# HarborC/PL-SLAM

Hardware: NVIDIA H100
Metric: frames/sec (extract+match+pose-LM) 640x480 (higher is better)
Workload: dtype u8/i32 front-end, f32 descriptors, f64 LM

## Files before the change

pl-slam_b200/csrc/match.cu:

```cuda

#include "common.cuh"
#include "search.cuh"
#include "libm_glibc.cuh"
#include <vector>

namespace pl {

constexpr int GC = 64, GR = 48, NCELL = GC * GR, HISTO = 30;

__device__ __forceinline__ int hamming256(const uint8_t* a, const uint8_t* b) {
  const uint4* pa = reinterpret_cast<const uint4*>(a);
  const uint4* pb = reinterpret_cast<const uint4*>(b);
  uint4 a0 = pa[0], a1 = pa[1], b0 = pb[0], b1 = pb[1];
  return __popc(a0.x ^ b0.x) + __popc(a0.y ^ b0.y) + __popc(a0.z ^ b0.z) + __popc(a0.w ^ b0.w) +
         __popc(a1.x ^ b1.x) + __popc(a1.y ^ b1.y) + __popc(a1.z ^ b1.z) + __popc(a1.w ^ b1.w);
}

__device__ __forceinline__ unsigned long long warp_min_u64(unsigned long long v) {
#pragma unroll
  for (int o = 16; o > 0; o >>= 1) {
    unsigned long long t = __shfl_xor_sync(0xffffffffu, v, o);
    v = t < v ? t : v;
  }
  return v;
}

struct GridP { float minX, minY, maxX, maxY, invW, invH; };
__host__ __device__ inline GridP make_grid(const float* b) {
  GridP g;
  g.minX = b[0]; g.minY = b[1]; g.maxX = b[2]; g.maxY = b[3];
  g.invW = (float)GC / (g.maxX - g.minX);
  g.invH = (float)GR / (g.maxY - g.minY);
  return g;
}

__device__ void build_point_grid(const PLKeyPoint* keys, int n, const GridP& g, unsigned short* start,
                                 unsigned short* fill, unsigned short* items, int lane) {
  for (int i = lane; i < NCELL; i += 32) fill[i] = 0;
  __syncwarp();
  for (int i0 = 0; i0 < n; i0 += 32) {
    int i = i0 + lane, c = -1;
    if (i < n) {
      int px = (int)roundf(__fmul_rn(__fsub_rn(keys[i].x, g.minX), g.invW));
      int py = (int)roundf(__fmul_rn(__fsub_rn(keys[i].y, g.minY), g.invH));
      if (px >= 0 && px < GC && py >= 0 && py < GR) c = px * GR + py;
    }
    unsigned peers = __match_any_sync(0xffffffffu, c);
    if (c >= 0 && (peers & ((1u << lane) - 1u)) == 0) fill[c] += (unsigned short)__popc(peers);
    __syncwarp();
  }
  int run = 0;
  for (int c0 = 0; c0 < NCELL; c0 += 32) {
    int v = fill[c0 + lane], incl = v;
#pragma unroll
    for (int o = 1; o < 32; o <<= 1) { int t = __shfl_up_sync(0xffffffffu, incl, o); if (lane >= o) incl += t; }
    start[c0 + lane] = (unsigned short)(run + incl - v);
    run += __shfl_sync(0xffffffffu, incl, 31);
  }
  if (lane == 0) start[NCELL] = (unsigned short)run;
  __syncwarp();
  for (int i = lane; i < NCELL; i += 32) fill[i] = 0;
  __syncwarp();
  for (int i0 = 0; i0 < n; i0 += 32) {
    int i = i0 + lane, c = -1;
    if (i < n) {
      int px = (int)roundf(__fmul_rn(__fsub_rn(keys[i].x, g.minX), g.invW));
      int py = (int)roundf(__fmul_rn(__fsub_rn(keys[i].y, g.minY), g.invH));
      if (px >= 0 && px < GC && py >= 0 && py < GR) c = px * GR + py;
    }
    unsigned peers = __match_any_sync(0xffffffffu, c);
    unsigned lt = peers & ((1u << lane) - 1u);
    if (c >= 0) items[start[c] + fill[c] + __popc(lt)] = (unsigned short)i;
    __syncwarp();
    if (c >= 0 && lt == 0) fill[c] += (unsigned short)__popc(peers);
    __syncwarp();
  }
}

struct Window { int x0, x1, y0, y1; bool ok; };
__device__ __forceinline__ Window make_window(const GridP& g, float x, float y, float r) {
  Window w;
  w.ok = false;
  w.x0 = max(0, (int)floorf(__fmul_rn(__fsub_rn(__fsub_rn(x, g.minX), r), g.invW)));
  if (w.x0 >= GC) return w;
  w.x1 = min(GC - 1, (int)ceilf(__fmul_rn(__fadd_rn(__fsub_rn(x, g.minX), r), g.invW)));
  if (w.x1 < 0) return w;
  w.y0 = max(0, (int)floorf(__fmul_rn(__fsub_rn(__fsub_rn(y, g.minY), r), g.invH)));
  if (w.y0 >= GR) return w;
  w.y1 = min(GR - 1, (int)ceilf(__fmul_rn(__fadd_rn(__fsub_rn(y, g.minY), r), g.invH)));
  if (w.y1 < 0) return w;
  w.ok = true;
  return w;
}

__device__ __forceinline__ unsigned long long mk_key(int dist, int c, int j, int idx) {
  return ((unsigned long long)dist << 52) | ((unsigned long long)c << 40) | ((unsigned long long)j << 20) |
         (unsigned long long)idx;
}
constexpr unsigned long long KEY_NONE = ~0ull;
__device__ __forceinline__ int key_dist(unsigned long long k) { return (int)(k >> 52); }
__device__ __forceinline__ int key_idx(unsigned long long k) { return (int)(k & 0xfffff); }

struct Top2 { unsigned long long best, second; };

constexpr int kPackShift = 11, kPackIdMask = (1 << kPackShift) - 1, kPackMaxKeys = 1 << kPackShift;
__device__ __forceinline__ bool pack_octaves(const PLKeyPoint* keys, int n, int nitems, unsigned short* items, int lane) {
  if (n > kPackMaxKeys) return false;
  for (int j = lane; j < nitems; j += 32) {
    const int id = items[j];
    items[j] = (unsigned short)(id | ((keys[id].octave & 31) << kPackShift));
  }
  __syncwarp();
  return true;
}

template <typename Skip>
__device__ __forceinline__ Top2 window_top2(const PLKeyPoint* keys, const uint8_t* desc, const unsigned short* start,
                                            const unsigned short* items, const GridP& g, float x, float y, float r,
                                            int minLevel, int maxLevel, const uint8_t* q, Skip skip, int lane,
                                            bool packed = false) {
  Top2 t;
  t.best = KEY_NONE; t.second = KEY_NONE;
  Window w = make_window(g, x, y, r);
  if (!w.ok) return t;
  const bool checkLevels = (minLevel > 0) || (maxLevel >= 0);
  const int ncy = w.y1 - w.y0 + 1, ncell = (w.x1 - w.x0 + 1) * ncy;
  unsigned long long k1 = KEY_NONE, k2 = KEY_NONE;
  const int q32 = 32 / ncy, r32 = 32 - q32 * ncy;
  int cx = lane / ncy, cy = lane - cx * ncy;
  for (int c = lane; c < ncell; c += 32, cx += q32, cy += r32) {
    if (cy >= ncy) { cy -= ncy; cx++; }
    const int ix = w.x0 + cx, iy = w.y0 + cy;
    int cb = start[ix * GR + iy], ce = start[ix * GR + iy + 1];
    for (int j = cb; j < ce; j++) {
      const int it = items[j];
      const int id = packed ? (it & kPackIdMask) : it;
      if (checkLevels) {
        const int oct = packed ? (it >> kPackShift) : keys[id].octave;
        if (oct < minLevel) continue;
        if (maxLevel >= 0 && oct > maxLevel) continue;
      }
      const PLKeyPoint& kp = keys[id];
      if (!(fabsf(__fsub_rn(kp.x, x)) < r && fabsf(__fsub_rn(kp.y, y)) < r)) continue;
      int dist = hamming256(q, desc + 32 * id);
      if (skip(id, dist)) continue;
      unsigned long long k = mk_key(dist, c, j - cb, id);
      if (k < k1) { k2 = k1; k1 = k; }
      else if (k < k2) k2 = k;
    }
  }
  t.best = warp_min_u64(k1);
  t.second = warp_min_u64(k1 == t.best ? k2 : k1);
  return t;
}

__device__ void three_maxima(const int* cnt, int& ind1, int& ind2, int& ind3) {
  int max1 = 0, max2 = 0, max3 = 0;
  ind1 = ind2 = ind3 = -1;
  for (int i = 0; i < HISTO; i++) {
    const int s = cnt[i];
    if (s > max1) { max3 = max2; max2 = max1; max1 = s; ind3 = ind2; ind2 = ind1; ind1 = i; }
    else if (s > max2) { max3 = max2; max2 = s; ind3 = ind2; ind2 = i; }
    else if (s > max3) { max3 = s; ind3 = i; }
  }
  if ((float)max2 < __fmul_rn(0.1f, (float)max1)) { ind2 = -1; ind3 = -1; }
  else if ((float)max3 < __fmul_rn(0.1f, (float)max1)) { ind3 = -1; }
}
__device__ __forceinline__ int rot_bin(float a1, float a2) {
  float rot = __fsub_rn(a1, a2);
  if (rot < 0.0f) rot = __fadd_rn(rot, 360.0f);
  int bin = (int)roundf(__fmul_rn(rot, 1.0f / HISTO));
  if (bin == HISTO) bin = 0;
  return bin;
}

struct SmemGrid {
  unsigned short* start; unsigned short* fill; unsigned short* items;
};
__device__ __forceinline__ SmemGrid carve_grid(unsigned char* smem, int cap) {
  SmemGrid s;
  s.start = reinterpret_cast<unsigned short*>(smem);
  s.fill = s.start + NCELL + 2;
  s.items = s.fill + NCELL;
  (void)cap;
  return s;
}
static size_t grid_smem_bytes(int cap) { return (size_t)(NCELL + 2 + NCELL + cap) * 2; }

__global__ void __launch_bounds__(32) k_assign_grid(const PLKeyPoint* keys, const int* n, int cap, const float* bounds,
                                                    int* out_start, int* out_items) {
  extern __shared__ unsigned char smem[];
  const int b = blockIdx.x, lane = threadIdx.x;
  SmemGrid sg = carve_grid(smem, cap);
  GridP g = make_grid(bounds);
  const int nn = min(n[b], cap);
  build_point_grid(keys + (long long)b * cap, nn, g, sg.start, sg.fill, sg.items, lane);
  __syncwarp();
  for (int i = lane; i <= NCELL; i += 32) out_start[(long long)b * (NCELL + 1) + i] = sg.start[i];
  for (int i = lane; i < sg.start[NCELL]; i += 32) out_items[(long long)b * cap + i] = sg.items[i];
}

struct SkipInit {
  const int* matchedDist;
  __device__ bool operator()(int id, int dist) const { return matchedDist[id] <= dist; }
};

__global__ void __launch_bounds__(32) k_search_init(const PLKeyPoint* keys1, const uint8_t* desc1, const int* n1,
                                                    const PLKeyPoint* keys2, const uint8_t* desc2, const int* n2,
                                                    int cap, const float* bounds, float* prev_matched, int* matches12,
                                                    int* nmatches_out, int windowSize, float nnratio, int checkOri,
                                                    int* scratch ) {
  extern __shared__ unsigned char smem[];
  __shared__ int hist[HISTO];
  const int b = blockIdx.x, lane = threadIdx.x;
  SmemGrid sg = carve_grid(smem, cap);
  GridP g = make_grid(bounds);
  const PLKeyPoint* k1 = keys1 + (long long)b * cap;
  const PLKeyPoint* k2 = keys2 + (long long)b * cap;
  const uint8_t* d1 = desc1 + (long long)b * cap * 32;
  const uint8_t* d2 = desc2 + (long long)b * cap * 32;
  const int N1 = min(n1[b], cap), N2 = min(n2[b], cap);
  float* pm = prev_matched + (long long)b * cap * 2;
  int* m12 = matches12 + (long long)b * cap;
  int* matchedDist = scratch + (long long)b * 2 * cap;
  int* m21 = matchedDist + cap;
  build_point_grid(k2, N2, g, sg.start, sg.fill, sg.items, lane);
  const bool packed = pack_octaves(k2, N2, sg.start[NCELL], sg.items, lane);
  for (int i = lane; i < N1; i += 32) m12[i] = -1;
  for (int i = lane; i < N2; i += 32) { matchedDist[i] = 0x7fffffff; m21[i] = -1; }
  if (lane < HISTO) hist[lane] = 0;
  __syncwarp();
  unsigned char* bins = reinterpret_cast<unsigned char*>(sg.fill);
  for (int i = lane; i < N1; i += 32) bins[i] = 255;
  __syncwarp();
  int nmatches = 0;
  SkipInit skip{matchedDist};
  for (int i1 = 0; i1 < N1; i1++) {
    if (k1[i1].octave > 0) continue;
    Top2 t = window_top2(k2, d2, sg.start, sg.items, g, pm[2 * i1], pm[2 * i1 + 1], (float)windowSize, 0, 0,
                         d1 + 32 * i1, skip, lane, packed);
    if (t.best == KEY_NONE) continue;
    const int bestDist = key_dist(t.best), bestIdx2 = key_idx(t.best);
    const float bestDist2 = (t.second == KEY_NONE) ? 2147483648.0f : (float)key_dist(t.second);
    if (bestDist <= 50 && (float)bestDist < __fmul_rn(bestDist2, nnratio)) {
      int old = m21[bestIdx2];
      __syncwarp();
      if (old >= 0) nmatches--;
      nmatches++;
      if (lane == 0) {
        if (old >= 0) m12[old] = -1;
        m12[i1] = bestIdx2;
        m21[bestIdx2] = i1;
        matchedDist[bestIdx2] = bestDist;
        if (checkOri) { int bin = rot_bin(k1[i1].angle, k2[bestIdx2].angle); bins[i1] = (unsigned char)bin; hist[bin]++; }
      }
      __syncwarp();
    }
  }
  if (checkOri) {
    int i1m, i2m, i3m;
    three_maxima(hist, i1m, i2m, i3m);
    int removed = 0;
    for (int i = lane; i < N1; i += 32) {
      int bin = bins[i];
      if (bin != 255 && bin != i1m && bin != i2m && bin != i3m && m12[i] >= 0) { m12[i] = -1; removed++; }
    }
    nmatches -= warp_sum(removed);
  }
  __syncwarp();
  for (int i = lane; i < N1; i += 32)
    if (m12[i] >= 0) { pm[2 * i] = k2[m12[i]].x; pm[2 * i + 1] = k2[m12[i]].y; }
  if (lane == 0) nmatches_out[b] = nmatches;
}

struct SkipAssigned {
  const int* match;
  __device__ bool operator()(int id, int) const { return match[id] != -1; }
};

struct ProjLastArgs {
  const PLKeyPoint* keys; const uint8_t* desc; const int* n; int cap;
  const float* bounds; const float* Tcw; const float* K; const float* scaleFactors; int nlevels;
  const int* n_last; int cap_last; const uint8_t* last_valid; const float* last_pos; const uint8_t* last_desc;
  const int* last_octave; const float* last_angle;
  float th; int checkOri; const uint8_t* preassigned; int* match; int* nmatches;
  int kfMode = 0, maxDist = 100; const float *min_dist = nullptr, *max_dist = nullptr; float Ow[3] = {0, 0, 0}; float logSF = 1.f;
  const int* gate = nullptr; int gate_min = 0;
  const int* last_row = nullptr;
};

__global__ void __launch_bounds__(32) k_search_proj_last(ProjLastArgs A) {
  extern __shared__ unsigned char smem[];
  __shared__ int hist[HISTO];
  const int b = blockIdx.x, lane = threadIdx.x;
  if (A.gate && A.gate[b] >= A.gate_min) return;
  SmemGrid sg = carve_grid(smem, A.cap);
  GridP g = make_grid(A.bounds);
  const PLKeyPoint* kc = A.keys + (long long)b * A.cap;
  const uint8_t* dc = A.desc + (long long)b * A.cap * 32;
  const int N = min(A.n[b], A.cap), NL = min(A.n_last[b], A.cap_last);
  int* match = A.match + (long long)b * A.cap;
  const float* T = A.Tcw + 16 * b;
  const long long lb = (long long)b * A.cap_last;
  build_point_grid(kc, N, g, sg.start, sg.fill, sg.items, lane);
  const bool packed = pack_octaves(kc, N, sg.start[NCELL], sg.items, lane);
  for (int i = lane; i < N; i += 32) match[i] = (A.preassigned && A.preassigned[(long long)b * A.cap + i]) ? -2 : -1;
  if (lane < HISTO) hist[lane] = 0;
  unsigned char* bins = reinterpret_cast<unsigned char*>(sg.fill);
  __syncwarp();
  for (int i = lane; i < N; i += 32) bins[i] = 255;
  __syncwarp();
  int nmatches = 0;
  SkipAssigned skip{match};
  const float* Kb = A.K + 4 * b;
  const float fx = Kb[0], fy = Kb[1], cx = Kb[2], cy = Kb[3];
  for (int i = 0; i < NL; i++) {
    if (!A.last_valid[lb + i]) continue;
    const long long row = A.last_row ? (long long)A.last_row[lb + i] : lb + i;
    const float* X = A.last_pos + row * 3;
    float xc = __fadd_rn(__fadd_rn(__fadd_rn(__fmul_rn(T[0], X[0]), __fmul_rn(T[1], X[1])), __fmul_rn(T[2], X[2])), T[3]);
    float yc = __fadd_rn(__fadd_rn(__fadd_rn(__fmul_rn(T[4], X[0]), __fmul_rn(T[5], X[1])), __fmul_rn(T[6], X[2])), T[7]);
    float zc = __fadd_rn(__fadd_rn(__fadd_rn(__fmul_rn(T[8], X[0]), __fmul_rn(T[9], X[1])), __fmul_rn(T[10], X[2])), T[11]);
    const float invzc = (float)(1.0 / (double)zc);
    if (!A.kfMode && invzc < 0) continue;
    float u = __fadd_rn(__fmul_rn(__fmul_rn(fx, xc), invzc), cx);
    float v = __fadd_rn(__fmul_rn(__fmul_rn(fy, yc), invzc), cy);
    if (u < g.minX || u > g.maxX) continue;
    if (v < g.minY || v > g.maxY) continue;
    int oct;
    if (A.kfMode) {
      const float p0 = __fsub_rn(X[0], A.Ow[0]), p1 = __fsub_rn(X[1], A.Ow[1]), p2 = __fsub_rn(X[2], A.Ow[2]);
      const float dist3D = (float)sqrt((double)p0 * p0 + (double)p1 * p1 + (double)p2 * p2);
      if (dist3D < __fmul_rn(0.8f, A.min_dist[lb + i]) || dist3D > __fmul_rn(1.2f, A.max_dist[lb + i])) continue;
      const float ratio = __fdiv_rn(A.max_dist[lb + i], dist3D);
      oct = (int)ceilf(__fdiv_rn(glibc::logf_(ratio), A.logSF));
      if (oct < 0) oct = 0; else if (oct >= A.nlevels) oct = A.nlevels - 1;
    } else oct = A.last_octave[lb + i];
    const float radius = __fmul_rn(A.th, A.scaleFactors[oct]);
    Top2 t = window_top2(kc, dc, sg.start, sg.items, g, u, v, radius, oct - 1, oct + 1, A.last_desc + row * 32,
                         skip, lane, packed);
    if (t.best == KEY_NONE) continue;
    const int bestDist = key_dist(t.best), bestIdx2 = key_idx(t.best);
    if (bestDist <= A.maxDist) {
      nmatches++;
      if (lane == 0) {
        match[bestIdx2] = i;
        if (A.checkOri) { int bin = rot_bin(A.last_angle[lb + i], kc[bestIdx2].angle); bins[bestIdx2] = (unsigned char)bin; hist[bin]++; }
      }
      __syncwarp();
    }
  }
  if (A.checkOri) {
    int i1m, i2m, i3m;
    three_maxima(hist, i1m, i2m, i3m);
    int removed = 0;
    for (int i = lane; i < N; i += 32) {
      int bin = bins[i];
      if (bin != 255 && bin != i1m && bin != i2m && bin != i3m) { match[i] = -1; removed++; }
    }
    nmatches -= warp_sum(removed);
  }
  if (lane == 0) A.nmatches[b] = nmatches;
}

struct ProjPointsArgs {
  const PLKeyPoint* keys; const uint8_t* desc; const int* n; int cap;
  const float* bounds; const float* scaleFactors;
  const int* n_mp; int cap_mp; const uint8_t* in_view; const float* proj; const int* level; const float* view_cos;
  const uint8_t* mp_desc; float th; float nnratio; const uint8_t* preassigned; int* match; int* nmatches;
  const float* th_frame;
  const int* desc_row;
};

__global__ void __launch_bounds__(32) k_search_proj_points(ProjPointsArgs A) {
  extern __shared__ unsigned char smem[];
  const int b = blockIdx.x, lane = threadIdx.x;
  SmemGrid sg = carve_grid(smem, A.cap);
  GridP g = make_grid(A.bounds);
  const PLKeyPoint* k = A.keys + (long long)b * A.cap;
  const uint8_t* d = A.desc + (long long)b * A.cap * 32;
  const int N = min(A.n[b], A.cap), NM = min(A.n_mp[b], A.cap_mp);
  int* match = A.match + (long long)b * A.cap;
  const long long mb = (long long)b * A.cap_mp;
  build_point_grid(k, N, g, sg.start, sg.fill, sg.items, lane);
  const bool packed = pack_octaves(k, N, sg.start[NCELL], sg.items, lane);
  for (int i = lane; i < N; i += 32) match[i] = (A.preassigned && A.preassigned[(long long)b * A.cap + i]) ? -2 : -1;
  __syncwarp();
  int nmatches = 0;
  SkipAssigned skip{match};
  const float th = A.th_frame ? A.th_frame[b] : A.th;
  const bool bFactor = th != 1.0f;
  for (int i = 0; i < NM; i++) {
    if (!A.in_view[mb + i]) continue;
    const int lvl = A.level[mb + i];
    float r = ((double)A.view_cos[mb + i] > 0.998) ? 2.5f : 4.0f;
    if (bFactor) r = __fmul_rn(r, th);
    const long long drow = A.desc_row ? (long long)A.desc_row[mb + i] : mb + i;
    Top2 t = window_top2(k, d, sg.start, sg.items, g, A.proj[(mb + i) * 2], A.proj[(mb + i) * 2 + 1],
                         __fmul_rn(r, A.scaleFactors[lvl]), lvl - 1, lvl, A.mp_desc + drow * 32, skip, lane, packed);
    if (t.best == KEY_NONE) continue;
    const int bestDist = key_dist(t.best), bestIdx = key_idx(t.best);
    if (bestDist <= 100) {
      if (t.second != KEY_NONE) {
        const int bestDist2 = key_dist(t.second);
        if (k[bestIdx].octave == k[key_idx(t.second)].octave && (float)bestDist > __fmul_rn(A.nnratio, (float)bestDist2))
          continue;
      }
      nmatches++;
      if (lane == 0) match[bestIdx] = i;
      __syncwarp();
    }
  }
  if (lane == 0) A.nmatches[b] = nmatches;
}

__device__ __forceinline__ void knn2_row(const uint8_t* q, const uint8_t* train, int n2, int lane, int& i0, int& d0,
                                         int& i1, int& d1v) {
  unsigned long long k1 = KEY_NONE, k2 = KEY_NONE;
  for (int t = lane; t < n2; t += 32) {
    unsigned long long k = ((unsigned long long)hamming256(q, train + 32 * t) << 32) | (unsigned)t;
    if (k < k1) { k2 = k1; k1 = k; } else if (k < k2) k2 = k;
  }
  unsigned long long b = warp_min_u64(k1);
  unsigned long long s = warp_min_u64(k1 == b ? k2 : k1);
  i0 = b == KEY_NONE ? -1 : (int)(b & 0xffffffffu); d0 = b == KEY_NONE ? -1 : (int)(b >> 32);
  i1 = s == KEY_NONE ? -1 : (int)(s & 0xffffffffu); d1v = s == KEY_NONE ? -1 : (int)(s >> 32);
}

__global__ void __launch_bounds__(128) k_bf_knn2(const uint8_t* d1, const int* n1, const uint8_t* d2, const int* n2,
                                                 int cap1, int cap2, int* idx, int* dist) {
  const int b = blockIdx.y, lane = threadIdx.x & 31, q = blockIdx.x * 4 + (threadIdx.x >> 5);
  const int N1 = min(n1[b], cap1), N2 = min(n2[b], cap2);
  if (q >= N1) return;
  int i0, dd0, i1, dd1;
  knn2_row(d1 + ((long long)b * cap1 + q) * 32, d2 + (long long)b * cap2 * 32, N2, lane, i0, dd0, i1, dd1);
  if (lane == 0) {
    long long o = ((long long)b * cap1 + q) * 2;
    idx[o] = i0; idx[o + 1] = i1; dist[o] = dd0; dist[o + 1] = dd1;
  }
}

__device__ void frame_bf_match_cta(const uint8_t* da, int na, const uint8_t* db, int nb, float TH, float nnratio,
                                   short* m, short* bd0, short* bd1, int* hist ) {
  const int tid = threadIdx.x, lane = tid & 31, wid = tid >> 5;
  for (int i = tid; i < na; i += 128) m[i] = -1;
  for (int i = tid; i < 257; i += 128) hist[i] = 0;
  __syncthreads();
  if (na < 1 || nb < 2) return;
  for (int q = wid; q < na; q += 4) {
    int i0, d0, i1, d1;
    knn2_row(da + 32 * q, db, nb, lane, i0, d0, i1, d1);
    if (lane == 0) { m[q] = (short)i0; bd0[q] = (short)d0; bd1[q] = (short)d1; atomicAdd(&hist[d1 - d0], 1); }
  }
  __syncthreads();
  __shared__ int s_med, s_mad;
  if (tid == 0) {
    int need = na / 2, acc = 0, v = 256;
    for (; v >= 0; v--) { acc += hist[v]; if (acc > need) break; }
    s_med = v;
  }
  __syncthreads();
  const int med = s_med;
  for (int i = tid; i < 257; i += 128) hist[i] = 0;
  __syncthreads();
  for (int q = tid; q < na; q += 128) atomicAdd(&hist[abs((int)bd1[q] - (int)bd0[q] - med)], 1);
  __syncthreads();
  if (tid == 0) {
    int need = na / 2, acc = 0, v = 0;
    for (; v <= 256; v++) { acc += hist[v]; if (acc > need) break; }
    s_mad = v;
  }
  __syncthreads();
  const double nn12_th = 1.4826 * (double)(float)s_mad * 0.5;
  for (int q = tid; q < na; q += 128) {
    const float d0 = (float)bd0[q], d1 = (float)bd1[q];
    const double dist_12 = (double)(d1 - d0);
    if (!(dist_12 > nn12_th && d0 < TH && d0 < __fmul_rn(nnratio, d1))) m[q] = -1;
  }
  __syncthreads();
}

__global__ void __launch_bounds__(128) k_search_double(const uint8_t* d1, const int* n1, const uint8_t* d2,
                                                       const int* n2, int cap1, int cap2, float TH, float nnratio,
                                                       int mutual, int* matches, int* nmatches) {
  extern __shared__ unsigned char smem[];
  __shared__ int hist[257];
  const int b = blockIdx.x, tid = threadIdx.x;
  const int N1 = min(n1[b], cap1), N2 = min(n2[b], cap2);
  short* m1 = reinterpret_cast<short*>(smem);
  short* m2 = m1 + cap1;
  short* bd0 = m2 + cap2;
  short* bd1 = bd0 + max(cap1, cap2);
  const uint8_t* a = d1 + (long long)b * cap1 * 32;
  const uint8_t* c = d2 + (long long)b * cap2 * 32;
// ... 192 lines not shown
      __syncwarp();
    }
  }
  if (lane == 0) A.nmatches[b] = nmatches;
}

struct TriArgs {
  const PLKeyPoint *k1, *k2; const uint8_t *d1, *d2, *mp1, *mp2;
  const int *q_idx1, *q_s, *q_e, *fv2_items; int nq, n1;
  float F[9], ex, ey; const float *scale2, *sigma2_2; int checkOri;
  int* matches12; int* nmatches; unsigned char* bins;
};
__global__ void __launch_bounds__(256) k_search_triangulation(TriArgs A) {
  __shared__ int hist[HISTO];
  __shared__ int s_nm, s_keep[3];
  const int tid = threadIdx.x;
  if (tid < HISTO) hist[tid] = 0;
  if (tid == 0) s_nm = 0;
  for (int i = tid; i < A.n1; i += blockDim.x) { A.matches12[i] = -1; A.bins[i] = 255; }
  __syncthreads();
  for (int q = tid; q < A.nq; q += blockDim.x) {
    const int idx1 = A.q_idx1[q];
    if (A.mp1[idx1]) continue;
    const PLKeyPoint kp1 = A.k1[idx1];
    const float la = __fadd_rn(__fadd_rn(__fmul_rn(kp1.x, A.F[0]), __fmul_rn(kp1.y, A.F[3])), A.F[6]);
    const float lb = __fadd_rn(__fadd_rn(__fmul_rn(kp1.x, A.F[1]), __fmul_rn(kp1.y, A.F[4])), A.F[7]);
    const float lc = __fadd_rn(__fadd_rn(__fmul_rn(kp1.x, A.F[2]), __fmul_rn(kp1.y, A.F[5])), A.F[8]);
    const float den = __fadd_rn(__fmul_rn(la, la), __fmul_rn(lb, lb));
    int bestDist = 50, bestIdx2 = -1;
    for (int i2 = A.q_s[q]; i2 < A.q_e[q]; i2++) {
      const int idx2 = A.fv2_items[i2];
      if (A.mp2[idx2]) continue;
      const int dist = hamming256(A.d1 + 32 * idx1, A.d2 + 32 * idx2);
      if (dist > 50 || dist > bestDist) continue;
      const PLKeyPoint kp2 = A.k2[idx2];
      const float dx = __fsub_rn(A.ex, kp2.x), dy = __fsub_rn(A.ey, kp2.y);
      if (__fadd_rn(__fmul_rn(dx, dx), __fmul_rn(dy, dy)) < __fmul_rn(100.f, A.scale2[kp2.octave])) continue;
      const float num = __fadd_rn(__fadd_rn(__fmul_rn(la, kp2.x), __fmul_rn(lb, kp2.y)), lc);
      if (den == 0.f) continue;
      const float dsqr = __fdiv_rn(__fmul_rn(num, num), den);
      if ((double)dsqr < 3.84 * (double)A.sigma2_2[kp2.octave]) { bestIdx2 = idx2; bestDist = dist; }
    }
    if (bestIdx2 >= 0) {
      A.matches12[idx1] = bestIdx2;
      atomicAdd(&s_nm, 1);
      if (A.checkOri) { const int bin = rot_bin(kp1.angle, A.k2[bestIdx2].angle); A.bins[idx1] = (unsigned char)bin; atomicAdd(&hist[bin], 1); }
    }
  }
  __syncthreads();
  if (A.checkOri) {
    if (tid == 0) { int a, b, c; three_maxima(hist, a, b, c); s_keep[0] = a; s_keep[1] = b; s_keep[2] = c; }
    __syncthreads();
    for (int i = tid; i < A.n1; i += blockDim.x) {
      const int bin = A.bins[i];
      if (bin != 255 && bin != s_keep[0] && bin != s_keep[1] && bin != s_keep[2]) { A.matches12[i] = -1; atomicSub(&s_nm, 1); }
    }
    __syncthreads();
  }
  if (tid == 0) *A.nmatches = s_nm;
}

struct FuseArgs {
  const PLKeyPoint* keys; const uint8_t* desc; int n; float bounds[4]; float T[16], Ow[3], K[4];
  const float *scaleFactors, *invSigma2; float logScaleFactor; int nLevels;
  int n_mp; const uint8_t* skip; const float *pos, *normal, *minDist, *maxDist; const uint8_t* mp_desc; float th;
  int *best_idx, *best_dist;
};
struct SkipChi2 {
  const PLKeyPoint* k; const float* inv; float u, v;
  __device__ bool operator()(int id, int) const {
    const float ex = __fsub_rn(u, k[id].x), ey = __fsub_rn(v, k[id].y);
    const float e2 = __fadd_rn(__fmul_rn(ex, ex), __fmul_rn(ey, ey));
    return (double)__fmul_rn(e2, inv[k[id].octave]) > 5.99;
  }
};
constexpr int kFuseWarps = 16;
__global__ void __launch_bounds__(32 * kFuseWarps) k_fuse_search(FuseArgs A) {
  extern __shared__ unsigned char smem[];
  const int lane = threadIdx.x & 31, wid = threadIdx.x >> 5;
  SmemGrid sg = carve_grid(smem, A.n);
  const GridP g = make_grid(A.bounds);
  __shared__ int s_packed;
  if (wid == 0) {
    build_point_grid(A.keys, A.n, g, sg.start, sg.fill, sg.items, lane);
    const bool pk = pack_octaves(A.keys, A.n, sg.start[NCELL], sg.items, lane);
    if (lane == 0) s_packed = pk;
  }
  __syncthreads();
  const bool packed = s_packed != 0;
  for (int i = wid; i < A.n_mp; i += kFuseWarps) {
    int bi = -1, bd = 256;
    bool go = !(A.skip && A.skip[i]);
    float u = 0.f, v = 0.f; int lvl = 0;
    if (go) {
      const float P[3] = {A.pos[3 * i], A.pos[3 * i + 1], A.pos[3 * i + 2]};
      float Pc[3];
      for (int r = 0; r < 3; r++)
        Pc[r] = __fadd_rn(__fadd_rn(__fadd_rn(__fmul_rn(A.T[4 * r], P[0]), __fmul_rn(A.T[4 * r + 1], P[1])), __fmul_rn(A.T[4 * r + 2], P[2])), A.T[4 * r + 3]);
      go = !(Pc[2] < 0.0f);
      if (go) {
        const float invz = __fdiv_rn(1.0f, Pc[2]);
        u = __fadd_rn(__fmul_rn(A.K[0], __fmul_rn(Pc[0], invz)), A.K[2]);
        v = __fadd_rn(__fmul_rn(A.K[1], __fmul_rn(Pc[1], invz)), A.K[3]);
        go = (u >= A.bounds[0] && u < A.bounds[2] && v >= A.bounds[1] && v < A.bounds[3]);
      }
      if (go) {
        const float PO[3] = {__fsub_rn(P[0], A.Ow[0]), __fsub_rn(P[1], A.Ow[1]), __fsub_rn(P[2], A.Ow[2])};
        const float dist3D = (float)sqrt((double)PO[0] * PO[0] + (double)PO[1] * PO[1] + (double)PO[2] * PO[2]);
        go = !(dist3D < __fmul_rn(0.8f, A.minDist[i]) || dist3D > __fmul_rn(1.2f, A.maxDist[i]));
        if (go) {
          const double dot = (double)PO[0] * A.normal[3 * i] + (double)PO[1] * A.normal[3 * i + 1] + (double)PO[2] * A.normal[3 * i + 2];
          go = !(dot < 0.5 * (double)dist3D);
          const float ratio = __fdiv_rn(A.maxDist[i], dist3D);
          lvl = (int)ceilf(__fdiv_rn(glibc::logf_(ratio), A.logScaleFactor));
          if (lvl < 0) lvl = 0; else if (lvl >= A.nLevels) lvl = A.nLevels - 1;
        }
      }
    }
    if (go) {
      SkipChi2 skip{A.keys, A.invSigma2, u, v};
      const Top2 t = window_top2(A.keys, A.desc, sg.start, sg.items, g, u, v, __fmul_rn(A.th, A.scaleFactors[lvl]), lvl - 1, lvl,
                                 A.mp_desc + 32 * (long long)i, skip, lane, packed);
      if (t.best != KEY_NONE) { bi = key_idx(t.best); bd = key_dist(t.best); }
    }
    if (lane == 0) { A.best_idx[i] = bi; A.best_dist[i] = bd; }
  }
}

struct BowArgs {
  const PLKeyPoint *kK, *kF; const uint8_t *dK, *dF, *mpK;
  const int *pairK_s, *pairK_e, *pairF_s, *pairF_e, *itK, *itF; int npairs, nF;
  float nnratio; int checkOri;
  int* matchesF; unsigned char* bins; int* nmatches;
  const uint8_t* mpF = nullptr;
  int strict = 0;
};
constexpr int kBowWarps = 16;
__global__ void __launch_bounds__(32 * kBowWarps) k_search_by_bow(BowArgs A) {
  __shared__ int hist[HISTO];
  __shared__ int s_nm, s_keep[3];
  const int tid = threadIdx.x, lane = tid & 31, wid = tid >> 5;
  if (tid < HISTO) hist[tid] = 0;
  if (tid == 0) s_nm = 0;
  for (int j = tid; j < A.nF; j += blockDim.x) { A.matchesF[j] = -1; A.bins[j] = 255; }
  __syncthreads();
  for (int p = wid; p < A.npairs; p += kBowWarps) {
    const int fs = A.pairF_s[p], fe = A.pairF_e[p];
    for (int iK = A.pairK_s[p]; iK < A.pairK_e[p]; iK++) {
      const int idxK = A.itK[iK];
      if (!A.mpK[idxK]) continue;
      unsigned long long k1 = KEY_NONE, k2 = KEY_NONE;
      for (int c = fs + lane; c < fe; c += 32) {
        const int idxF = A.itF[c];
        if (A.matchesF[idxF] >= 0) continue;
        if (A.mpF && !A.mpF[idxF]) continue;
        const int dist = hamming256(A.dK + 32 * idxK, A.dF + 32 * idxF);
        const unsigned long long k = mk_key(dist, 0, c - fs, idxF);
        if (k < k1) { k2 = k1; k1 = k; } else if (k < k2) k2 = k;
      }
      const unsigned long long best = warp_min_u64(k1);
      const unsigned long long second = warp_min_u64(k1 == best ? k2 : k1);
      if (best == KEY_NONE) continue;
      const int bestDist1 = key_dist(best), bestIdxF = key_idx(best);
      const int bestDist2 = (second == KEY_NONE) ? 256 : key_dist(second);
      if ((A.strict ? bestDist1 < 50 : bestDist1 <= 50) && (float)bestDist1 < __fmul_rn(A.nnratio, (float)bestDist2)) {
        if (lane == 0) {
          A.matchesF[bestIdxF] = idxK;
// ... 679 lines not shown
```

Before: 12260.

## Batch per-query window searches across warp lanes with speculative conflict re-search

Replaces the per-query warp-cooperative window search in the init, projection and map-point search kernels with a lane-per-query search over batches of 32 queries. The sequential matching commit is then replayed in order, and a query is re-searched warp-wide only when its best or second candidate was taken earlier in the same batch. Separately, the grid build drops the separate fill array by reusing start as a cursor and shifting it back afterwards, which shrinks shared memory and adds a dedicated bins region. The intent is to remove per-query warp underutilisation, since windows are small; the cost is lane divergence from uneven window sizes and extra redundant searches when conflicts occur.

```diff
diff --git a/pl-slam_b200/csrc/match.cu b/pl-slam_b200/csrc/match.cu
--- a/pl-slam_b200/csrc/match.cu
+++ b/pl-slam_b200/csrc/match.cu
@@ -34,24 +34,24 @@
   return g;
 }
 
-__device__ void build_point_grid(const PLKeyPoint* keys, int n, const GridP& g, unsigned short* start,
-                                 unsigned short* fill, unsigned short* items, int lane) {
-  for (int i = lane; i < NCELL; i += 32) fill[i] = 0;
+__device__ __forceinline__ int grid_cell(const PLKeyPoint& k, const GridP& g) {
+  const int px = (int)roundf(__fmul_rn(__fsub_rn(k.x, g.minX), g.invW));
+  const int py = (int)roundf(__fmul_rn(__fsub_rn(k.y, g.minY), g.invH));
+  return (px >= 0 && px < GC && py >= 0 && py < GR) ? px * GR + py : -1;
+}
+__device__ void build_point_grid(const PLKeyPoint* keys, int n, const GridP& g, unsigned short* start, unsigned short* items,
+                                 int lane) {
+  for (int i = lane; i < NCELL; i += 32) start[i] = 0;
   __syncwarp();
   for (int i0 = 0; i0 < n; i0 += 32) {
-    int i = i0 + lane, c = -1;
-    if (i < n) {
-      int px = (int)roundf(__fmul_rn(__fsub_rn(keys[i].x, g.minX), g.invW));
-      int py = (int)roundf(__fmul_rn(__fsub_rn(keys[i].y, g.minY), g.invH));
-      if (px >= 0 && px < GC && py >= 0 && py < GR) c = px * GR + py;
-    }
+    const int i = i0 + lane, c = i < n ? grid_cell(keys[i], g) : -1;
     unsigned peers = __match_any_sync(0xffffffffu, c);
-    if (c >= 0 && (peers & ((1u << lane) - 1u)) == 0) fill[c] += (unsigned short)__popc(peers);
+    if (c >= 0 && (peers & ((1u << lane) - 1u)) == 0) start[c] += (unsigned short)__popc(peers);
     __syncwarp();
   }
   int run = 0;
   for (int c0 = 0; c0 < NCELL; c0 += 32) {
-    int v = fill[c0 + lane], incl = v;
+    int v = start[c0 + lane], incl = v;
 #pragma unroll
     for (int o = 1; o < 32; o <<= 1) { int t = __shfl_up_sync(0xffffffffu, incl, o); if (lane >= o) incl += t; }
     start[c0 + lane] = (unsigned short)(run + incl - v);
@@ -59,22 +59,23 @@
   }
   if (lane == 0) start[NCELL] = (unsigned short)run;
   __syncwarp();
-  for (int i = lane; i < NCELL; i += 32) fill[i] = 0;
-  __syncwarp();
   for (int i0 = 0; i0 < n; i0 += 32) {
-    int i = i0 + lane, c = -1;
-    if (i < n) {
-      int px = (int)roundf(__fmul_rn(__fsub_rn(keys[i].x, g.minX), g.invW));
-      int py = (int)roundf(__fmul_rn(__fsub_rn(keys[i].y, g.minY), g.invH));
-      if (px >= 0 && px < GC && py >= 0 && py < GR) c = px * GR + py;
-    }
+    const int i = i0 + lane, c = i < n ? grid_cell(keys[i], g) : -1;
     unsigned peers = __match_any_sync(0xffffffffu, c);
     unsigned lt = peers & ((1u << lane) - 1u);
-    if (c >= 0) items[start[c] + fill[c] + __popc(lt)] = (unsigned short)i;
+    if (c >= 0) items[start[c] + __popc(lt)] = (unsigned short)i;
     __syncwarp();
-    if (c >= 0 && lt == 0) fill[c] += (unsigned short)__popc(peers);
+    if (c >= 0 && lt == 0) start[c] += (unsigned short)__popc(peers);
     __syncwarp();
   }
+  for (int c0 = NCELL - 31; c0 >= 1; c0 -= 32) {
+    const unsigned short v = start[c0 + lane - 1];
+    __syncwarp();
+    start[c0 + lane] = v;
+    __syncwarp();
+  }
+  if (lane == 0) start[0] = 0;
+  __syncwarp();
 }
 
 struct Window { int x0, x1, y0, y1; bool ok; };
@@ -154,6 +155,50 @@
   return t;
 }
 
+
+__device__ __forceinline__ int hamming256(const uint4& a0, const uint4& a1, const uint8_t* b) {
+  const uint4* pb = reinterpret_cast<const uint4*>(b);
+  uint4 b0 = pb[0], b1 = pb[1];
+  return __popc(a0.x ^ b0.x) + __popc(a0.y ^ b0.y) + __popc(a0.z ^ b0.z) + __popc(a0.w ^ b0.w) +
+         __popc(a1.x ^ b1.x) + __popc(a1.y ^ b1.y) + __popc(a1.z ^ b1.z) + __popc(a1.w ^ b1.w);
+}
+
+template <typename Skip>
+__device__ __forceinline__ Top2 lane_top2(const PLKeyPoint* keys, const uint8_t* desc, const unsigned short* start,
+                                          const unsigned short* items, const GridP& g, bool ok, float x, float y, float r,
+                                          int minLevel, int maxLevel, const uint8_t* q, Skip skip, bool packed) {
+  Top2 t;
+  t.best = KEY_NONE; t.second = KEY_NONE;
+  const Window w = make_window(g, x, y, r);
+  if (!ok || !w.ok) return t;
+  const uint4 q0 = reinterpret_cast<const uint4*>(q)[0], q1 = reinterpret_cast<const uint4*>(q)[1];
+  const bool checkLevels = (minLevel > 0) || (maxLevel >= 0);
+  for (int ix = w.x0; ix <= w.x1; ix++) {
+    const int jb = start[ix * GR + w.y0], je = start[ix * GR + w.y1 + 1];
+    for (int j = jb; j < je; j++) {
+      const int it = items[j];
+      const int id = packed ? (it & kPackIdMask) : it;
+      if (checkLevels) {
+        const int oct = packed ? (it >> kPackShift) : keys[id].octave;
+        if (oct < minLevel) continue;
+        if (maxLevel >= 0 && oct > maxLevel) continue;
+      }
+      const PLKeyPoint& kp = keys[id];
+      if (!(fabsf(__fsub_rn(kp.x, x)) < r && fabsf(__fsub_rn(kp.y, y)) < r)) continue;
+      const int dist = hamming256(q0, q1, desc + 32 * id);
+      if (skip(id, dist)) continue;
+      const unsigned long long k = mk_key(dist, ix - w.x0, j, id);
+      if (k < t.best) { t.second = t.best; t.best = k; }
+      else if (k < t.second) t.second = k;
+    }
+  }
+  return t;
+}
+
+__device__ __forceinline__ bool taken_in_batch(int taken, int a, int b) {
+  return __any_sync(0xffffffffu, taken >= 0 && (taken == a || taken == b));
+}
+
 __device__ void three_maxima(const int* cnt, int& ind1, int& ind2, int& ind3) {
   int max1 = 0, max2 = 0, max3 = 0;
   ind1 = ind2 = ind3 = -1;
@@ -175,17 +220,16 @@
 }
 
 struct SmemGrid {
-  unsigned short* start; unsigned short* fill; unsigned short* items;
+  unsigned short* start; unsigned short* items; unsigned char* bins;
 };
 __device__ __forceinline__ SmemGrid carve_grid(unsigned char* smem, int cap) {
   SmemGrid s;
   s.start = reinterpret_cast<unsigned short*>(smem);
-  s.fill = s.start + NCELL + 2;
-  s.items = s.fill + NCELL;
-  (void)cap;
+  s.items = s.start + NCELL + 2;
+  s.bins = reinterpret_cast<unsigned char*>(s.items + cap);
   return s;
 }
-static size_t grid_smem_bytes(int cap) { return (size_t)(NCELL + 2 + NCELL + cap) * 2; }
+static size_t grid_smem_bytes(int cap) { return (size_t)(NCELL + 2 + cap) * 2 + cap; }
 
 __global__ void __launch_bounds__(32) k_assign_grid(const PLKeyPoint* keys, const int* n, int cap, const float* bounds,
                                                     int* out_start, int* out_items) {
@@ -194,7 +238,7 @@
   SmemGrid sg = carve_grid(smem, cap);
   GridP g = make_grid(bounds);
   const int nn = min(n[b], cap);
-  build_point_grid(keys + (long long)b * cap, nn, g, sg.start, sg.fill, sg.items, lane);
+  build_point_grid(keys + (long long)b * cap, nn, g, sg.start, sg.items, lane);
   __syncwarp();
   for (int i = lane; i <= NCELL; i += 32) out_start[(long long)b * (NCELL + 1) + i] = sg.start[i];
   for (int i = lane; i < sg.start[NCELL]; i += 32) out_items[(long long)b * cap + i] = sg.items[i];
@@ -224,38 +268,61 @@
   int* m12 = matches12 + (long long)b * cap;
   int* matchedDist = scratch + (long long)b * 2 * cap;
   int* m21 = matchedDist + cap;
-  build_point_grid(k2, N2, g, sg.start, sg.fill, sg.items, lane);
+  build_point_grid(k2, N2, g, sg.start, sg.items, lane);
   const bool packed = pack_octaves(k2, N2, sg.start[NCELL], sg.items, lane);
   for (int i = lane; i < N1; i += 32) m12[i] = -1;
   for (int i = lane; i < N2; i += 32) { matchedDist[i] = 0x7fffffff; m21[i] = -1; }
   if (lane < HISTO) hist[lane] = 0;
   __syncwarp();
-  unsigned char* bins = reinterpret_cast<unsigned char*>(sg.fill);
+  unsigned char* bins = sg.bins;
   for (int i = lane; i < N1; i += 32) bins[i] = 255;
   __syncwarp();
   int nmatches = 0;
   SkipInit skip{matchedDist};
-  for (int i1 = 0; i1 < N1; i1++) {
-    if (k1[i1].octave > 0) continue;
-    Top2 t = window_top2(k2, d2, sg.start, sg.items, g, pm[2 * i1], pm[2 * i1 + 1], (float)windowSize, 0, 0,
-                         d1 + 32 * i1, skip, lane, packed);
-    if (t.best == KEY_NONE) continue;
-    const int bestDist = key_dist(t.best), bestIdx2 = key_idx(t.best);
-    const float bestDist2 = (t.second == KEY_NONE) ? 2147483648.0f : (float)key_dist(t.second);
-    if (bestDist <= 50 && (float)bestDist < __fmul_rn(bestDist2, nnratio)) {
-      int old = m21[bestIdx2];
-      __syncwarp();
-      if (old >= 0) nmatches--;
-      nmatches++;
-      if (lane == 0) {
-        if (old >= 0) m12[old] = -1;
-        m12[i1] = bestIdx2;
-        m21[bestIdx2] = i1;
-        matchedDist[bestIdx2] = bestDist;
-        if (checkOri) { int bin = rot_bin(k1[i1].angle, k2[bestIdx2].angle); bins[i1] = (unsigned char)bin; hist[bin]++; }
+  const float r = (float)windowSize;
+  for (int base = 0; base < N1; base += 32) {
+    const int qi = base + lane;
+    const bool ok = qi < N1 && k1[qi].octave <= 0;
+    const float qx = ok ? pm[2 * qi] : 0.f, qy = ok ? pm[2 * qi + 1] : 0.f;
+    const Top2 t = lane_top2(k2, d2, sg.start, sg.items, g, ok, qx, qy, r, 0, 0, d1 + 32 * (long long)qi, skip, packed);
+    int old = -1, bin = 0;
+    if (t.best != KEY_NONE) {
+      old = m21[key_idx(t.best)];
+      if (checkOri) bin = rot_bin(k1[qi].angle, k2[key_idx(t.best)].angle);
+    }
+    int taken = -1;
+    const int nq = min(32, N1 - base);
+    for (int j = 0; j < nq; j++) {
+      const int src = j, i1 = base + j;
+      if (!__shfl_sync(0xffffffffu, ok, src)) continue;
+      Top2 tj;
+      tj.best = __shfl_sync(0xffffffffu, t.best, src); tj.second = __shfl_sync(0xffffffffu, t.second, src);
+      int oldj = __shfl_sync(0xffffffffu, old, src), binj = __shfl_sync(0xffffffffu, bin, src);
+      if (taken_in_batch(taken, key_idx(tj.best), key_idx(tj.second))) {
+        tj = window_top2(k2, d2, sg.start, sg.items, g, pm[2 * i1], pm[2 * i1 + 1], r, 0, 0, d1 + 32 * i1, skip, lane, packed);
+        if (tj.best != KEY_NONE) {
+          oldj = m21[key_idx(tj.best)];
+          if (checkOri) binj = rot_bin(k1[i1].angle, k2[key_idx(tj.best)].angle);
+        }
       }
-      __syncwarp();
-    }
+      if (tj.best == KEY_NONE) continue;
+      const int bestDist = key_dist(tj.best), bestIdx2 = key_idx(tj.best);
+      const float bestDist2 = (tj.second == KEY_NONE) ? 2147483648.0f : (float)key_dist(tj.second);
+      if (bestDist <= 50 && (float)bestDist < __fmul_rn(bestDist2, nnratio)) {
+        if (oldj >= 0) nmatches--;
+        nmatches++;
+        if (lane == 0) {
+          if (oldj >= 0) m12[oldj] = -1;
+          m12[i1] = bestIdx2;
+          m21[bestIdx2] = i1;
+          matchedDist[bestIdx2] = bestDist;
+          if (checkOri) { bins[i1] = (unsigned char)binj; hist[binj]++; }
+        }
+        if (lane == j) taken = bestIdx2;
+        __syncwarp();
+      }
+    }
+    __syncwarp();
   }
   if (checkOri) {
     int i1m, i2m, i3m;
@@ -302,11 +369,11 @@
   int* match = A.match + (long long)b * A.cap;
   const float* T = A.Tcw + 16 * b;
   const long long lb = (long long)b * A.cap_last;
-  build_point_grid(kc, N, g, sg.start, sg.fill, sg.items, lane);
+  build_point_grid(kc, N, g, sg.start, sg.items, lane);
   const bool packed = pack_octaves(kc, N, sg.start[NCELL], sg.items, lane);
   for (int i = lane; i < N; i += 32) match[i] = (A.preassigned && A.preassigned[(long long)b * A.cap + i]) ? -2 : -1;
   if (lane < HISTO) hist[lane] = 0;
-  unsigned char* bins = reinterpret_cast<unsigned char*>(sg.fill);
+  unsigned char* bins = sg.bins;
   __syncwarp();
   for (int i = lane; i < N; i += 32) bins[i] = 255;
   __syncwarp();
@@ -314,41 +381,68 @@
   SkipAssigned skip{match};
   const float* Kb = A.K + 4 * b;
   const float fx = Kb[0], fy = Kb[1], cx = Kb[2], cy = Kb[3];
-  for (int i = 0; i < NL; i++) {
-    if (!A.last_valid[lb + i]) continue;
-    const long long row = A.last_row ? (long long)A.last_row[lb + i] : lb + i;
-    const float* X = A.last_pos + row * 3;
-    float xc = __fadd_rn(__fadd_rn(__fadd_rn(__fmul_rn(T[0], X[0]), __fmul_rn(T[1], X[1])), __fmul_rn(T[2], X[2])), T[3]);
-    float yc = __fadd_rn(__fadd_rn(__fadd_rn(__fmul_rn(T[4], X[0]), __fmul_rn(T[5], X[1])), __fmul_rn(T[6], X[2])), T[7]);
-    float zc = __fadd_rn(__fadd_rn(__fadd_rn(__fmul_rn(T[8], X[0]), __fmul_rn(T[9], X[1])), __fmul_rn(T[10], X[2])), T[11]);
-    const float invzc = (float)(1.0 / (double)zc);
-    if (!A.kfMode && invzc < 0) continue;
-    float u = __fadd_rn(__fmul_rn(__fmul_rn(fx, xc), invzc), cx);
-    float v = __fadd_rn(__fmul_rn(__fmul_rn(fy, yc), invzc), cy);
-    if (u < g.minX || u > g.maxX) continue;
-    if (v < g.minY || v > g.maxY) continue;
-    int oct;
-    if (A.kfMode) {
-      const float p0 = __fsub_rn(X[0], A.Ow[0]), p1 = __fsub_rn(X[1], A.Ow[1]), p2 = __fsub_rn(X[2], A.Ow[2]);
-      const float dist3D = (float)sqrt((double)p0 * p0 + (double)p1 * p1 + (double)p2 * p2);
-      if (dist3D < __fmul_rn(0.8f, A.min_dist[lb + i]) || dist3D > __fmul_rn(1.2f, A.max_dist[lb + i])) continue;
-      const float ratio = __fdiv_rn(A.max_dist[lb + i], dist3D);
-      oct = (int)ceilf(__fdiv_rn(glibc::logf_(ratio), A.logSF));
-      if (oct < 0) oct = 0; else if (oct >= A.nlevels) oct = A.nlevels - 1;
-    } else oct = A.last_octave[lb + i];
-    const float radius = __fmul_rn(A.th, A.scaleFactors[oct]);
-    Top2 t = window_top2(kc, dc, sg.start, sg.items, g, u, v, radius, oct - 1, oct + 1, A.last_desc + row * 32,
-                         skip, lane, packed);
-    if (t.best == KEY_NONE) continue;
-    const int bestDist = key_dist(t.best), bestIdx2 = key_idx(t.best);
-    if (bestDist <= A.maxDist) {
-      nmatches++;
-      if (lane == 0) {
-        match[bestIdx2] = i;
-        if (A.checkOri) { int bin = rot_bin(A.last_angle[lb + i], kc[bestIdx2].angle); bins[bestIdx2] = (unsigned char)bin; hist[bin]++; }
+  for (int base = 0; base < NL; base += 32) {
+    const int qi = base + lane;
+    bool ok = qi < NL && A.last_valid[lb + qi];
+    long long row = 0;
+    float u = 0.f, v = 0.f, radius = 0.f;
+    int oct = 0;
+    if (ok) {
+      row = A.last_row ? (long long)A.last_row[lb + qi] : lb + qi;
+      const float* X = A.last_pos + row * 3;
+      float xc = __fadd_rn(__fadd_rn(__fadd_rn(__fmul_rn(T[0], X[0]), __fmul_rn(T[1], X[1])), __fmul_rn(T[2], X[2])), T[3]);
+      float yc = __fadd_rn(__fadd_rn(__fadd_rn(__fmul_rn(T[4], X[0]), __fmul_rn(T[5], X[1])), __fmul_rn(T[6], X[2])), T[7]);
+      float zc = __fadd_rn(__fadd_rn(__fadd_rn(__fmul_rn(T[8], X[0]), __fmul_rn(T[9], X[1])), __fmul_rn(T[10], X[2])), T[11]);
+      const float invzc = (float)(1.0 / (double)zc);
+      u = __fadd_rn(__fmul_rn(__fmul_rn(fx, xc), invzc), cx);
+      v = __fadd_rn(__fmul_rn(__fmul_rn(fy, yc), invzc), cy);
+      if (!A.kfMode && invzc < 0) ok = false;
+      else if (u < g.minX || u > g.maxX || v < g.minY || v > g.maxY) ok = false;
+      else if (A.kfMode) {
+        const float p0 = __fsub_rn(X[0], A.Ow[0]), p1 = __fsub_rn(X[1], A.Ow[1]), p2 = __fsub_rn(X[2], A.Ow[2]);
+        const float dist3D = (float)sqrt((double)p0 * p0 + (double)p1 * p1 + (double)p2 * p2);
+        if (dist3D < __fmul_rn(0.8f, A.min_dist[lb + qi]) || dist3D > __fmul_rn(1.2f, A.max_dist[lb + qi])) ok = false;
+        else {
+          const float ratio = __fdiv_rn(A.max_dist[lb + qi], dist3D);
+          oct = (int)ceilf(__fdiv_rn(glibc::logf_(ratio), A.logSF));
+          if (oct < 0) oct = 0; else if (oct >= A.nlevels) oct = A.nlevels - 1;
+        }
+      } else oct = A.last_octave[lb + qi];
+      if (ok) radius = __fmul_rn(A.th, A.scaleFactors[oct]);
+    }
+    const Top2 t = lane_top2(kc, dc, sg.start, sg.items, g, ok, u, v, radius, oct - 1, oct + 1, A.last_desc + row * 32, skip,
+                              packed);
+    int bin = 0;
+    if (A.checkOri && t.best != KEY_NONE) bin = rot_bin(A.last_angle[lb + qi], kc[key_idx(t.best)].angle);
+    int taken = -1;
+    const int nq = min(32, NL - base);
+    for (int j = 0; j < nq; j++) {
+      const int src = j, i = base + j;
+      if (!__shfl_sync(0xffffffffu, ok, src)) continue;
+      unsigned long long best = __shfl_sync(0xffffffffu, t.best, src);
+      int binj = __shfl_sync(0xffffffffu, bin, src);
+      if (taken_in_batch(taken, key_idx(best), -1)) {
+        const float uj = __shfl_sync(0xffffffffu, u, src), vj = __shfl_sync(0xffffffffu, v, src);
+        const float rj = __shfl_sync(0xffffffffu, radius, src);
+        const int octj = __shfl_sync(0xffffffffu, oct, src);
+        const long long rowj = __shfl_sync(0xffffffffu, row, src);
+        best = window_top2(kc, dc, sg.start, sg.items, g, uj, vj, rj, octj - 1, octj + 1, A.last_desc + rowj * 32, skip, lane,
+                           packed).best;
+        if (A.checkOri && best != KEY_NONE) binj = rot_bin(A.last_angle[lb + i], kc[key_idx(best)].angle);
       }
-      __syncwarp();
-    }
+      if (best == KEY_NONE) continue;
+      const int bestDist = key_dist(best), bestIdx2 = key_idx(best);
+      if (bestDist <= A.maxDist) {
+        nmatches++;
+        if (lane == 0) {
+          match[bestIdx2] = i;
+          if (A.checkOri) { bins[bestIdx2] = (unsigned char)binj; hist[binj]++; }
+        }
+        if (lane == j) taken = bestIdx2;
+        __syncwarp();
+      }
+    }
+    __syncwarp();
   }
   if (A.checkOri) {
     int i1m, i2m, i3m;
@@ -382,7 +476,7 @@
   const int N = min(A.n[b], A.cap), NM = min(A.n_mp[b], A.cap_mp);
   int* match = A.match + (long long)b * A.cap;
   const long long mb = (long long)b * A.cap_mp;
-  build_point_grid(k, N, g, sg.start, sg.fill, sg.items, lane);
+  build_point_grid(k, N, g, sg.start, sg.items, lane);
   const bool packed = pack_octaves(k, N, sg.start[NCELL], sg.items, lane);
   for (int i = lane; i < N; i += 32) match[i] = (A.preassigned && A.preassigned[(long long)b * A.cap + i]) ? -2 : -1;
   __syncwarp();
@@ -390,26 +484,50 @@
   SkipAssigned skip{match};
   const float th = A.th_frame ? A.th_frame[b] : A.th;
   const bool bFactor = th != 1.0f;
-  for (int i = 0; i < NM; i++) {
-    if (!A.in_view[mb + i]) continue;
-    const int lvl = A.level[mb + i];
-    float r = ((double)A.view_cos[mb + i] > 0.998) ? 2.5f : 4.0f;
-    if (bFactor) r = __fmul_rn(r, th);
-    const long long drow = A.desc_row ? (long long)A.desc_row[mb + i] : mb + i;
-    Top2 t = window_top2(k, d, sg.start, sg.items, g, A.proj[(mb + i) * 2], A.proj[(mb + i) * 2 + 1],
-                         __fmul_rn(r, A.scaleFactors[lvl]), lvl - 1, lvl, A.mp_desc + drow * 32, skip, lane, packed);
-    if (t.best == KEY_NONE) continue;
-    const int bestDist = key_dist(t.best), bestIdx = key_idx(t.best);
-    if (bestDist <= 100) {
-      if (t.second != KEY_NONE) {
-        const int bestDist2 = key_dist(t.second);
-        if (k[bestIdx].octave == k[key_idx(t.second)].octave && (float)bestDist > __fmul_rn(A.nnratio, (float)bestDist2))
-          continue;
+  auto ratio_rejects = [&](const Top2& t) {
+    if (t.best == KEY_NONE || t.second == KEY_NONE) return false;
+    return k[key_idx(t.best)].octave == k[key_idx(t.second)].octave &&
+           (float)key_dist(t.best) > __fmul_rn(A.nnratio, (float)key_dist(t.second));
+  };
+  for (int base = 0; base < NM; base += 32) {
+    const int qi = base + lane;
+    const bool ok = qi < NM && A.in_view[mb + qi];
+    int lvl = 0;
+    long long drow = 0;
+    float x = 0.f, y = 0.f, rs = 0.f;
+    if (ok) {
+      lvl = A.level[mb + qi];
+      float r = ((double)A.view_cos[mb + qi] > 0.998) ? 2.5f : 4.0f;
+      if (bFactor) r = __fmul_rn(r, th);
+      rs = __fmul_rn(r, A.scaleFactors[lvl]);
+      drow = A.desc_row ? (long long)A.desc_row[mb + qi] : mb + qi;
+      x = A.proj[(mb + qi) * 2]; y = A.proj[(mb + qi) * 2 + 1];
+    }
+    const Top2 t = lane_top2(k, d, sg.start, sg.items, g, ok, x, y, rs, lvl - 1, lvl, A.mp_desc + drow * 32, skip, packed);
+    const bool rej = ratio_rejects(t);
+    int taken = -1;
+    const int nq = min(32, NM - base);
+    for (int j = 0; j < nq; j++) {
+      const int src = j, i = base + j;
+      if (!__shfl_sync(0xffffffffu, ok, src)) continue;
+      Top2 tj;
+      tj.best = __shfl_sync(0xffffffffu, t.best, src); tj.second = __shfl_sync(0xffffffffu, t.second, src);
+      bool rejj = __shfl_sync(0xffffffffu, rej, src);
+      if (taken_in_batch(taken, key_idx(tj.best), key_idx(tj.second))) {
+        const float xj = __shfl_sync(0xffffffffu, x, src), yj = __shfl_sync(0xffffffffu, y, src);
+        const float rj = __shfl_sync(0xffffffffu, rs, src);
+        const int lj = __shfl_sync(0xffffffffu, lvl, src);
+        const long long dj = __shfl_sync(0xffffffffu, drow, src);
+        tj = window_top2(k, d, sg.start, sg.items, g, xj, yj, rj, lj - 1, lj, A.mp_desc + dj * 32, skip, lane, packed);
+        rejj = ratio_rejects(tj);
       }
+      if (tj.best == KEY_NONE || key_dist(tj.best) > 100 || rejj) continue;
       nmatches++;
-      if (lane == 0) match[bestIdx] = i;
+      if (lane == 0) match[key_idx(tj.best)] = i;
+      if (lane == j) taken = key_idx(tj.best);
       __syncwarp();
     }
+    __syncwarp();
   }
   if (lane == 0) A.nmatches[b] = nmatches;
 }
@@ -768,7 +886,7 @@
   const GridP g = make_grid(A.bounds);
   __shared__ int s_packed;
   if (wid == 0) {
-    build_point_grid(A.keys, A.n, g, sg.start, sg.fill, sg.items, lane);
+    build_point_grid(A.keys, A.n, g, sg.start, sg.items, lane);
     const bool pk = pack_octaves(A.keys, A.n, sg.start[NCELL], sg.items, lane);
     if (lane == 0) s_packed = pk;
   }
```

Result: faster. 12970, median of 6 (+5.8%).
